# Sachin-A/TraceWeaver

Measured on AMD Instinct MI355X. Metric: spans/sec reconstructed + assignment accuracy vs ground truth, higher is better.
Workload: dtype int64 timestamps, f64 scores; 1 GPU; media_microservices shape (6 services, E in {1,1,1,1,2,4}), 100000 requests/service x 16 replicas per GPU, concurrency 1.6, two-pass reconstruction, device mixture refit; spans_per_gpu=25600000, spans_total=25600000, parallelism=units sharded, 1 rank(s), backend none

## Files before the change

include/traceweaver_amd.h:

```cpp
#ifndef TRACEWEAVER_AMD_H
#define TRACEWEAVER_AMD_H

#include <stdint.h>

#ifdef __cplusplus
extern "C" {
#endif

#define TW_MAX_EP 8
#define TW_TOPK 5
#define TW_MAX_COMP 5
#define TW_MAX_WINDOW 32
#define TW_CAND_WORDS 2
#define TW_SKIP_BASE 1024
#define TW_SKIP_STRIDE 128

typedef enum {
    TW_OK = 0,
    TW_ERR_ARG = -1,
    TW_ERR_UNSUPPORTED = -2,
    TW_ERR_DEVICE = -3,
    TW_ERR_STATE = -4,
    TW_ERR_WINDOW_WIDTH = -5,
    TW_ERR_WINDOW_SIZE = -6,
// ... 50 lines not shown
    int64_t gaps_count;
    int32_t device;
} tw_device_view;
int tw_device_buffers(tw_engine *e, tw_device_view *out);
int tw_set_gaps_device(tw_engine *e, const double *dev_gaps);

int tw_set_mixtures(tw_engine *e, const int32_t *mix_n, const double *mix_p);

#define TW_FIT_ROW_TAPE 34
int tw_fit_mixtures(tw_engine *e);
int tw_fit_mixtures_seeded(tw_engine *e, const uint32_t *unit_seed);
int tw_set_fit_seed(tw_engine *e, uint32_t seed);
int tw_fit_rows(tw_engine *e, int32_t *max_n);
int tw_fit_mixtures_tape(tw_engine *e, const double *tape, int64_t tape_len, const int64_t *slot_off);

int tw_get_mixtures(tw_engine *e, int32_t *mix_n, double *mix_p);

int tw_run_pass2(tw_engine *e);

typedef struct {
    int32_t *parent;
    int32_t *topk_idx;
    double *topk_score;
    int32_t *topk_n;
    int32_t *chosen;
    int64_t *leaves;
    uint8_t *window_end;
    int64_t *unit_stats;
} tw_results;
int tw_get_results(tw_engine *e, int pass, const tw_results *r);
// ... 187 lines not shown
```

traceweaver_amd/_ffi.py:

```python
import ctypes
import os

_HERE = os.path.dirname(os.path.abspath(__file__))
DEFAULT_LIB = os.path.join(_HERE, "lib", "libtwgpu.so")

TW_MAX_EP = 8
TW_TOPK = 5
TW_MAX_COMP = 5

STATUS = {0: "TW_OK", -1: "TW_ERR_ARG", -2: "TW_ERR_UNSUPPORTED", -3: "TW_ERR_DEVICE", -4: "TW_ERR_STATE",
          -5: "TW_ERR_WINDOW_WIDTH", -6: "TW_ERR_WINDOW_SIZE", -7: "TW_ERR_NAN_PARAMS", -8: "TW_ERR_SKIP_PARAMS",
          -9: "TW_ERR_SKIP_REFERENCE_RAISES"}
TW_SKIP_BASE = 1024
TW_SKIP_STRIDE = 128

c_i32p = ctypes.POINTER(ctypes.c_int32)
c_i64p = ctypes.POINTER(ctypes.c_int64)
c_u8p = ctypes.POINTER(ctypes.c_uint8)
c_f64p = ctypes.POINTER(ctypes.c_double)


class Batch(ctypes.Structure):
    _fields_ = [
        ("n_units", ctypes.c_int32),
# ... 92 lines not shown

class ClassProfile(ctypes.Structure):
    _fields_ = [(k, ctypes.c_void_p) for k in (
        "rows", "span_time", "span_min", "span_max", "self_time", "path_time", "path_rows", "path_trees", "offset",
        "class_counted", "class_latency", "class_path_time", "class_top_entry")]


TW_TREE_CONFIDENT = 8
TW_CONF_MAX_EDGES = 15
TW_DIST_MAX_Q = 32
TW_DIST_MAX_EDGES = 63
TW_CMP_MAX_Q = 8
TW_CMP_MAX_PAIRS = 64

EXPORTS = ["tw_create", "tw_destroy", "tw_last_error", "tw_load_batch", "tw_run_pass1", "tw_get_gaps", "tw_set_gaps",
           "tw_device_buffers", "tw_set_gaps_device", "tw_set_mixtures", "tw_fit_mixtures", "tw_fit_mixtures_seeded", "tw_set_fit_seed", "tw_fit_rows", "tw_fit_mixtures_tape", "tw_get_mixtures", "tw_run_pass2", "tw_get_results", "tw_get_gauss_params", "tw_get_timing",
           "tw_assign_service", "tw_find_order", "tw_order_bound", "tw_order_stage", "tw_order_load", "tw_set_truth", "tw_evaluate", "tw_measure_hbm_copy", "tw_host_alloc", "tw_host_free", "tw_build_distributions", "tw_scale_load", "tw_run_baseline", "tw_wap5_delays", "tw_wap5_parents",
           "tw_set_span_rows", "tw_set_parents", "tw_stitch_traces", "tw_set_row_groups", "tw_attribute_traces",
           "tw_get_decisions", "tw_score_traces", "tw_set_row_cohorts", "tw_latency_distributions", "tw_compare_cohorts", "tw_trace_signatures", "tw_class_profiles",
           "tw_corpus_create", "tw_corpus_destroy", "tw_corpus_last_error", "tw_corpus_add_files", "tw_corpus_set_callers", "tw_corpus_counts",
           "tw_corpus_string", "tw_corpus_loop_origin", "tw_corpus_trace_names", "tw_corpus_span_table", "tw_corpus_build_units"]


def load(path=None):
    path = path or DEFAULT_LIB
    if os.environ.get("TW_SET_HW_QUEUES", "0") not in ("", "0"):
        os.environ.setdefault("GPU_MAX_HW_QUEUES", "12")
    if not os.path.exists(path):
        raise ImportError(
            "traceweaver_amd: %s is missing -- build it with `python -c 'import __graft_entry__ as g; g.build()'` "
            "(hipcc --offload-arch=gfx950).  There is no CPU fallback." % path)
# ... 9 lines not shown
    lib.tw_get_gaps.argtypes = [vp, vp]
    lib.tw_set_gaps.argtypes = [vp, vp]
    lib.tw_run_baseline.argtypes = [vp, ctypes.c_int, vp]
    lib.tw_wap5_delays.argtypes = [vp, vp, vp, vp]
    lib.tw_wap5_parents.argtypes = [vp, vp, vp, vp]
    lib.tw_device_buffers.argtypes = [vp, ctypes.POINTER(DeviceView)]
    lib.tw_set_gaps_device.argtypes = [vp, vp]
    lib.tw_scale_load.argtypes = [vp, vp, vp, vp, vp, vp]
    lib.tw_set_mixtures.argtypes = [vp, vp, vp]
    lib.tw_run_pass2.argtypes = [vp]
    lib.tw_fit_mixtures.argtypes = [vp]
    lib.tw_fit_mixtures_seeded.argtypes = [vp, vp]
    lib.tw_set_fit_seed.argtypes = [vp, ctypes.c_uint32]
    lib.tw_fit_rows.argtypes = [vp, vp]
    lib.tw_fit_mixtures_tape.argtypes = [vp, vp, ctypes.c_int64, vp]
    lib.tw_get_mixtures.argtypes = [vp, vp, vp]
    lib.tw_get_results.argtypes = [vp, ctypes.c_int, ctypes.POINTER(Results)]
    lib.tw_get_gauss_params.argtypes = [vp, vp]
    lib.tw_get_timing.argtypes = [vp, vp, ctypes.c_int32]
    lib.tw_assign_service.argtypes = [vp, ctypes.c_int32, vp, vp, ctypes.c_int32, vp, vp, vp, vp, vp, vp, vp,
                                      ctypes.POINTER(Results)]
    lib.tw_find_order.argtypes = [vp, ctypes.c_int32, vp, vp, vp, vp, vp, vp, vp]
    lib.tw_order_bound.argtypes = [vp, ctypes.c_int32, vp, vp, vp, vp, vp, vp, vp, vp]
    lib.tw_order_stage.argtypes = [vp, ctypes.POINTER(Batch)]
    lib.tw_order_load.argtypes = [vp, ctypes.c_int32, vp, vp]
    lib.tw_set_truth.argtypes = [vp, vp, vp, ctypes.c_int64]
    lib.tw_evaluate.argtypes = [vp, vp, vp, vp]
    lib.tw_measure_hbm_copy.argtypes = [vp, ctypes.c_int64, ctypes.c_int32, ctypes.POINTER(ctypes.c_double)]
    lib.tw_build_distributions.argtypes = [vp, ctypes.c_int64, vp, vp, vp, ctypes.c_int64, ctypes.c_int32, vp, vp]
    lib.tw_set_span_rows.argtypes = [vp, ctypes.c_int64, vp, vp, vp, vp, vp, vp]
# ... 34 lines not shown
```

traceweaver_amd/csrc/tw_engine.hip:

```cpp
#include <algorithm>
#include <chrono>
#include <cmath>
#include <cstdio>
#include <cstdlib>
#include <cstring>
#include <functional>
#include <string>
#include <type_traits>
#include <vector>

#include <hip/hip_runtime.h>
#include <rocprim/rocprim.hpp>

#include "traceweaver_amd.h"
#include "tw_kernels.h"
#include "tw_fit.h"
#include "tw_eval.h"
#include "tw_skip.h"
#include "tw_load.h"
#include "tw_baselines.h"
#include "tw_stitch.h"
#include "tw_attr.h"
#include "tw_conf.h"
#include "tw_dist.h"
// ... 27 lines not shown
    int block_params;
    int coop;
    int set_hw_queues;
    int pipeline;
    int sig_hash_bits;
    int debug_lists;
    int stage_min_tiles;
    int tile_sub;
    int lean_pool;
    int split_twins, defer_min_e, lean_min_e, lean_grid, tile_max_deep;
    int64_t part_slots_max;
    int part_budget_deep;
    int fit_sort;
    int stage_gate;
    int fit_spec;
};

Knobs read_knobs() {
    Knobs K;
    K.tile = std::min(std::max(env_int("TW_TILE", kTile), 1), kTile);
    K.tile_threads = std::min(std::max(env_int("TW_TILE_THREADS", 2), 1), 4);
    K.tile_single = env_int("TW_TILE_SINGLE", 1);
    K.tile_single_threads = std::min(std::max(env_int("TW_TILE_SINGLE_THREADS", 1), 1), 4);
    K.tile_pair = env_int("TW_TILE_PAIR", 1);
    K.tile_pair_threads = std::min(std::max(env_int("TW_TILE_PAIR_THREADS", 2), 1), 2);
    K.tile_rank = env_int("TW_TILE_RANK", 1) != 0 ? 1 : 0;
    K.block_params = env_int("TW_BLOCK_PARAMS", 1);
    K.coop = std::min(std::max(env_int("TW_COOP_THREADS", kCoop), 1), kCoop);
    K.set_hw_queues = env_int("TW_SET_HW_QUEUES", 0);
    K.pipeline = env_int("TW_CLASS_PIPELINE", 1);
    K.sig_hash_bits = std::min(std::max(env_int("TW_SIG_HASH_BITS", 64), 1), 64);
    K.debug_lists = env_int("TW_DEBUG_LISTS", 0);
    K.stage_min_tiles = env_int("TW_STAGE_MIN_TILES", 1024);
    K.tile_sub = std::max(env_int("TW_TILE_SUB", 8), 1);
    K.lean_pool = std::min(std::max(env_int("TW_LEAN_POOL", 512), 1), 4096);
    K.split_twins = env_int("TW_SPLIT_TWINS", 2);
    K.defer_min_e = env_int("TW_DEFER_MIN_E", 5);
    K.lean_min_e = env_int("TW_LEAN_MIN_E", 5);
    K.lean_grid = std::max(env_int("TW_LEAN_GRID", TW_LEAN_GRID), 1);
    K.tile_max_deep = std::min(std::max(env_int("TW_TILE_MAX_DEEP", kTileMax), 0), kTileMax);
    K.part_slots_max = (int64_t)std::max(env_int("TW_PART_SLOTS_MAX", 16 << 20), 1024);
    K.part_budget_deep = env_int("TW_PART_BUDGET_DEEP", 2);
    K.fit_sort = env_int("TW_FIT_SORT", 0);
    K.stage_gate = env_int("TW_STAGE_GATE", 1);
    K.fit_spec = env_int("TW_FIT_SPEC", 1) != 0 ? 1 : 0;
    return K;
}

struct Mt19937 {
    uint32_t mt[624];
    int idx = 624;
    explicit Mt19937(uint32_t seed = 0u) {
        mt[0] = seed;
        for (int i = 1; i < 624; i++) mt[i] = 1812433253u * (mt[i - 1] ^ (mt[i - 1] >> 30)) + (uint32_t)i;
    }
    uint32_t next() {
        if (idx >= 624) {
            for (int i = 0; i < 624; i++) {
                const uint32_t y = (mt[i] & 0x80000000u) | (mt[(i + 1) % 624] & 0x7fffffffu);
                mt[i] = mt[(i + 397) % 624] ^ (y >> 1) ^ ((y & 1u) ? 0x9908b0dfu : 0u);
// ... 56 lines not shown
    int32_t *fit_ustart = nullptr, *fit_row_n = nullptr, *fit_row_uniq = nullptr;
    double* fit_centres = nullptr;
    hipEvent_t fit_fork = nullptr, fit_join = nullptr;
    double *fit_spec_centres = nullptr, *fit_spec_p = nullptr;
    int32_t *fit_spec_failed = nullptr, *fit_spec_ctr = nullptr;
    int32_t fit_spec_count[2] = {0, 0};
    double *fit_tape = nullptr, *fit_tape100 = nullptr;
    int64_t* fit_tape_off = nullptr;
    int64_t fit_tape_cap = 0;
    bool fit_runs_pending = false;
    bool fit_prepared = false;
    int32_t hard_pass1[kMaxEp + 1] = {};
    int8_t wide_pass1[kMaxEp + 1] = {};
    int32_t split_pass1[kMaxEp + 1] = {};
    bool pass1_done = false;
    std::vector<int32_t> fit_max_n;
    bool fit_max_n_valid = false;
    Mt19937 fit_rng;
    uint32_t fit_seed = 0;
    int32_t* slot_unit = nullptr;
    int32_t* tile_ids = nullptr;
    int32_t* ctr = nullptr;
    int64_t ctr_round_ints = 0, ctr_pass_ints = 0;
    int32_t tile_cls_off[kMaxEp + 2] = {};
    BlockRef* blk_tab = nullptr;
    int32_t blk_cls_off[kMaxEp + 2] = {};
    uint32_t *seg_gap = nullptr, *seg_gap_end = nullptr, *seg_gap_dst = nullptr;
    unsigned long long *comp_a = nullptr, *comp_b = nullptr;
    int64_t comp_cap = 0, n_gap_scored = 0;
    int32_t *truth = nullptr, *in_trace = nullptr;
    uint8_t* trace_bad = nullptr;
    unsigned long long* eval_counts = nullptr;
// ... 828 lines not shown
    delete e;
}

const char* tw_last_error(const tw_engine* e) { return e ? e->err.c_str() : "null engine"; }

int tw_load_batch(tw_engine* e, const tw_batch* b, int spans_on_device) {
    if (e == nullptr || b == nullptr) return TW_ERR_ARG;
    HIPCHK(hipSetDevice(e->device));
    if (b->n_units <= 0) return fail(e, TW_ERR_ARG, "n_units must be positive");
    if (b->topk != TW_TOPK) return fail(e, TW_ERR_UNSUPPORTED, "topk must be 5 (traceweaver_v3.py:1109)");
    if (b->skip != nullptr && spans_on_device)
        return fail(e, TW_ERR_UNSUPPORTED, "a skip-mode batch takes its span arrays from host memory (spans_on_device = 0)");
    if (b->batch_size <= 0 || b->batch_size_mis <= 0) return fail(e, TW_ERR_ARG, "batch sizes must be positive");
    free_all(e);
    e->fit_rng = Mt19937(e->fit_seed);
    e->fit_prepared = false; e->fit_runs_pending = false; e->fit_max_n_valid = false;
    e->units.assign((size_t)b->n_units, UnitDev{});
    e->tiles.clear();
    e->gs_off_h.assign((size_t)b->n_units, 0);
    int64_t ie = 0, gp = 0, slots = 0, gaps = 0, epi = 0, dagi = 0;
    std::vector<uint32_t> seg_in((size_t)b->n_units + 1), seg_out;
    for (int u = 0; u < b->n_units; u++) {
        UnitDev& U = e->units[(size_t)u];
        const int E = b->unit_E[u];
        const int64_t n = b->unit_in_off[u + 1] - b->unit_in_off[u];
        if (E < 1 || E > TW_MAX_EP) return fail(e, TW_ERR_UNSUPPORTED, "unit has E outside [1, TW_MAX_EP]");
        if (n < 2) return fail(e, TW_ERR_ARG, "a unit needs at least 2 incoming spans (the reference raises on max([]) for 1, traceweaver_v3.py:1119)");
        if (n > (1 << 26)) return fail(e, TW_ERR_ARG, "unit too large (more than 2^26 incoming spans: the selection work lists address a window's first span in 26 bits)");
        U.in_off = b->unit_in_off[u];
        U.tscale = b->unit_time_scale != nullptr ? b->unit_time_scale[u] : 1.0;
        U.float_time = b->unit_time_scale != nullptr ? 1 : 0;
// ... 214 lines not shown
            D.part_used = c + o_pu; D.split_count = c + o_sc; D.err = c + o_err; D.unit_ndirty = c + o_nd;
            D.redo_count = c + o_rd; D.fb_count = c + o_fc; D.defer_refused = c + o_dr; D.fb_total = c + o_ft; D.pair_busy = c + o_pb; D.any_wide = c + o_aw;
            D.unit_stats = (int64_t*)(c + o_us);
        };
        if (e->arena_open) e->arena_req.emplace_back(place, ((size_t)at * sizeof(int32_t) + 255) / 256 * 256);
        else { DEV_ALLOC(e->ctr, at); place(e->ctr); }
    }
    DEV_ALLOC(P.heavy_unit, sel_cap); DEV_ALLOC(P.heavy_win, sel_cap);
    DEV_ALLOC(P.tiny_unit, sel_cap); DEV_ALLOC(P.tiny_win, sel_cap);
    DEV_ALLOC(P.rheavy_unit, sel_cap); DEV_ALLOC(P.rheavy_win, sel_cap); DEV_ALLOC(P.rtiny_unit, sel_cap); DEV_ALLOC(P.rtiny_win, sel_cap);
    DEV_ALLOC(P.hard_unit, sel_cap / (kBruteMax + 1) + 1 + kSelSlots); DEV_ALLOC(P.hard_win, sel_cap / (kBruteMax + 1) + 1 + kSelSlots);
    DEV_ALLOC(e->rank_in, n_in_total); DEV_ALLOC(e->rank_out, n_out_total);
    DEV_ALLOC(e->agg_pair, P.n_tiles); DEV_ALLOC(e->agg_i32, P.n_tiles); DEV_ALLOC(e->agg_i32b, P.n_tiles);
    DEV_ALLOC(e->seg_in, (int64_t)seg_in.size()); DEV_ALLOC(e->seg_out, (int64_t)seg_out.size());
    DEV_ALLOC(e->gaps_sorted, gaps); DEV_ALLOC(e->fit_models, slots * kMaxComp * kModelStride);
    DEV_ALLOC(e->fit_uval, gaps); DEV_ALLOC(e->fit_ustart, gaps); DEV_ALLOC(e->fit_row_n, slots); DEV_ALLOC(e->fit_row_uniq, slots);
    DEV_ALLOC(e->fit_tape, slots * kFitRowTape); DEV_ALLOC(e->fit_tape_off, slots); DEV_ALLOC(e->fit_tape100, kMaxComp * 13);
    e->fit_tape_cap = slots * kFitRowTape;
    DEV_ALLOC(e->fit_centres, slots * kMaxComp * (kMaxComp + 1));
    DEV_ALLOC(e->fit_spec_centres, slots * (kMaxComp + 1)); DEV_ALLOC(e->fit_spec_p, slots * kMaxComp * 3);
    DEV_ALLOC(e->fit_spec_failed, slots); DEV_ALLOC(e->fit_spec_ctr, 2);
    DEV_ALLOC(e->slot_unit, slots); DEV_ALLOC(e->slot_scored, slots);
    DEV_ALLOC(e->seg_gap, (int64_t)seg_gap_h.size()); DEV_ALLOC(e->seg_gap_end, (int64_t)seg_gap_end_h.size()); DEV_ALLOC(e->seg_gap_dst, (int64_t)seg_gap_dst_h.size());
    e->comp_cap = std::max(std::max(n_in_total, n_out_total), e->n_gap_scored);
    DEV_ALLOC(e->comp_a, e->comp_cap); DEV_ALLOC(e->comp_b, e->comp_cap);
    e->skip_mode = b->skip != nullptr;
    std::vector<int32_t> perm_h, pool_h;
    std::vector<int64_t> tw_h;
    std::vector<double> dist_h;
    std::vector<SkipUnitDev> skip_h;
    std::vector<int64_t> sk_tw_off, sk_pool_off, sk_dist_off;
    if (e->skip_mode) {
        perm_h.resize((size_t)n_out_total);
        for (int u = 0; u < b->n_units; u++) {
            const UnitDev& U = e->units[(size_t)u];
            const tw_skip_unit& K = b->skip[u];
// ... 3 lines not shown
                for (int64_t q = 0; q < m; q++) idx[(size_t)q] = (int32_t)q;
                std::stable_sort(idx.begin(), idx.end(), [&](int32_t x, int32_t y) { return b->out_start[a + x] < b->out_start[a + y]; });
                std::copy(idx.begin(), idx.end(), perm_h.begin() + a);
            }
            sk_tw_off.push_back((int64_t)tw_h.size()); sk_pool_off.push_back((int64_t)pool_h.size()); sk_dist_off.push_back((int64_t)dist_h.size());
            tw_h.insert(tw_h.end(), K.tw_start, K.tw_start + K.n_tw);
            pool_h.insert(pool_h.end(), K.pool, K.pool + (int64_t)U.E * K.n_tw);
            dist_h.insert(dist_h.end(), K.dist, K.dist + (int64_t)(U.E + 1) * (U.E + 1) * 2);
        }
        e->skip_fetch_n = (int64_t)pool_h.size();
        DEV_ALLOC(e->skip_units, b->n_units); DEV_ALLOC(e->skip_perm, n_out_total); DEV_ALLOC(e->skip_tw, (int64_t)tw_h.size());
        DEV_ALLOC(e->skip_pool, (int64_t)pool_h.size()); DEV_ALLOC(e->skip_dist, (int64_t)dist_h.size()); DEV_ALLOC(e->skip_fetch, e->skip_fetch_n);
    }
    rc = arena_commit(e);
    if (rc != TW_OK) return rc;
    if (e->skip_mode) {
        for (int u = 0; u < b->n_units; u++) {
            SkipUnitDev K{};
            K.perm = e->skip_perm; K.tw_start = e->skip_tw + sk_tw_off[(size_t)u]; K.pool = e->skip_pool + sk_pool_off[(size_t)u];
            K.dist = e->skip_dist + sk_dist_off[(size_t)u]; K.fetches = e->skip_fetch + sk_pool_off[(size_t)u]; K.n_tw = b->skip[u].n_tw;
            skip_h.push_back(K);
        }
        HIPCHK(hipMemcpyAsync(e->skip_units, skip_h.data(), sizeof(SkipUnitDev) * skip_h.size(), hipMemcpyHostToDevice, e->stream));
        HIPCHK(hipMemcpyAsync(e->skip_perm, perm_h.data(), sizeof(int32_t) * perm_h.size(), hipMemcpyHostToDevice, e->stream));
        HIPCHK(hipMemcpyAsync(e->skip_tw, tw_h.data(), sizeof(int64_t) * tw_h.size(), hipMemcpyHostToDevice, e->stream));
        HIPCHK(hipMemcpyAsync(e->skip_pool, pool_h.data(), sizeof(int32_t) * pool_h.size(), hipMemcpyHostToDevice, e->stream));
        HIPCHK(hipMemcpyAsync(e->skip_dist, dist_h.data(), sizeof(double) * dist_h.size(), hipMemcpyHostToDevice, e->stream));
        HIPCHK(hipStreamSynchronize(e->stream));
    }
    HIPCHK(hipMemsetAsync(P.prof, 0, sizeof(unsigned long long) * 32, e->stream));
// ... 26 lines not shown
    HIPCHK(hipMemsetAsync(P.tk_score, 0xff, sizeof(double) * (size_t)std::max<int64_t>(n_in_total * kTopK, 1), e->stream));
    HIPCHK(hipMemsetAsync(e->mix_n_dev, 0, sizeof(int32_t) * std::max<int64_t>(slots, 1), e->stream));
    HIPCHK(hipStreamSynchronize(e->stream));
    e->scaled_upload = b->unit_time_scale != nullptr;
    e->state = ST_LOADED; e->pass1_done = false;
    for (int E = 0; E <= kMaxEp; E++) { e->wide_pass1[E] = -1; e->hard_pass1[E] = -1; e->split_pass1[E] = -1; }
    return TW_OK;
}

int tw_run_pass1(tw_engine* e) {
    if (e == nullptr) return TW_ERR_ARG;
    if (e->state < ST_LOADED) return fail(e, TW_ERR_STATE, "tw_run_pass1 before tw_load_batch");
    HIPCHK(hipSetDevice(e->device));
    drop_forest(e);
    const int rc = run_pass(e, 1);
    e->fit_prepared = false; e->fit_runs_pending = false; e->fit_max_n_valid = false;
    if (rc == TW_OK) { e->state = ST_PASS1; e->pass1_done = true; }
    return rc;
}

int tw_get_gaps(tw_engine* e, double* gaps) {
    if (e == nullptr || gaps == nullptr) return TW_ERR_ARG;
    if (e->state != ST_PASS1) return fail(e, TW_ERR_STATE, "tw_get_gaps is valid right after tw_run_pass1");
    if (e->skip_mode) return fail(e, TW_ERR_STATE, "a skip-mode batch runs one pass (traceweaver_v3.py:1155-1156): there is no refit");
    HIPCHK(hipSetDevice(e->device));
    HIPCHK(hipMemcpyAsync(gaps, e->P.gaps, sizeof(double) * e->n_gaps, hipMemcpyDeviceToHost, e->stream));
    HIPCHK(hipStreamSynchronize(e->stream));
    return TW_OK;
}

int tw_set_gaps(tw_engine* e, const double* gaps) {
    if (e == nullptr || gaps == nullptr) return TW_ERR_ARG;
    if (e->state < ST_LOADED) return fail(e, TW_ERR_STATE, "tw_set_gaps before tw_load_batch");
    if (e->skip_mode) return fail(e, TW_ERR_STATE, "a skip-mode batch runs one pass (traceweaver_v3.py:1155-1156): there is no refit");
    HIPCHK(hipSetDevice(e->device));
    HIPCHK(hipMemcpyAsync(e->P.gaps, gaps, sizeof(double) * e->n_gaps, hipMemcpyHostToDevice, e->stream));
    HIPCHK(hipStreamSynchronize(e->stream));
    e->fit_prepared = false; e->fit_runs_pending = false; e->fit_max_n_valid = false;
    e->state = ST_PASS1;
    return TW_OK;
}

int tw_device_buffers(tw_engine* e, tw_device_view* out) {
    if (e == nullptr || out == nullptr) return TW_ERR_ARG;
    if (e->state < ST_LOADED) return fail(e, TW_ERR_STATE, "tw_device_buffers before tw_load_batch");
    out->parent = e->P.parent; out->parent_count = e->n_ie;
    out->gaps = e->P.gaps; out->gaps_count = e->n_gaps;
    out->device = e->device;
    return TW_OK;
}

int tw_set_gaps_device(tw_engine* e, const double* dev_gaps) {
    if (e == nullptr || dev_gaps == nullptr) return TW_ERR_ARG;
    if (e->state < ST_LOADED) return fail(e, TW_ERR_STATE, "tw_set_gaps_device before tw_load_batch");
    if (e->skip_mode) return fail(e, TW_ERR_STATE, "a skip-mode batch runs one pass (traceweaver_v3.py:1155-1156): there is no refit");
    HIPCHK(hipSetDevice(e->device));
    HIPCHK(hipMemcpyAsync(e->P.gaps, dev_gaps, sizeof(double) * e->n_gaps, hipMemcpyDeviceToDevice, e->stream));
    HIPCHK(hipStreamSynchronize(e->stream));
    e->fit_prepared = false; e->fit_runs_pending = false; e->fit_max_n_valid = false;
    e->state = ST_PASS1;
    return TW_OK;
}

int tw_set_mixtures(tw_engine* e, const int32_t* mix_n, const double* mix_p) {
    if (e == nullptr || mix_n == nullptr || mix_p == nullptr) return TW_ERR_ARG;
    if (e->state < ST_PASS1) return fail(e, TW_ERR_STATE, "tw_set_mixtures before tw_run_pass1");
    if (e->skip_mode) return fail(e, TW_ERR_STATE, "a skip-mode batch runs one pass (traceweaver_v3.py:1155-1156): there is no second pass");
    HIPCHK(hipSetDevice(e->device));
    for (int64_t q = 0; q < e->n_slots; q++)
        if (mix_n[q] < 0 || mix_n[q] > TW_MAX_COMP) return fail(e, TW_ERR_ARG, "mixture component count outside [0, TW_MAX_COMP]");
    HIPCHK(hipMemcpyAsync(e->mix_n_dev, mix_n, sizeof(int32_t) * e->n_slots, hipMemcpyHostToDevice, e->stream));
    HIPCHK(hipMemcpyAsync(e->mix_p_dev, mix_p, sizeof(double) * e->n_slots * kMaxComp * 3, hipMemcpyHostToDevice, e->stream));
    const int64_t total = e->n_slots * kMaxComp;
    hipLaunchKernelGGL(k_mix_consts, dim3((unsigned)((total + 255) / 256)), dim3(256), 0, e->stream, (const double*)e->mix_p_dev, (const int32_t*)e->mix_n_dev, (const int32_t*)e->slot_unit, e->P.units, e->mix_c_dev, total);
    HIPCHK(hipGetLastError());
    HIPCHK(hipStreamSynchronize(e->stream));
    e->state = ST_MIX;
    return TW_OK;
}

namespace {

FitDev fit_dev(tw_engine* e) {
    FitDev F{};
    F.units = e->P.units; F.n_units = e->P.n_units; F.n_slots = e->n_slots; F.gaps = e->P.gaps; F.sorted = e->gaps_sorted;
    F.gs_off = e->P.gs_off; F.slot_unit = e->slot_unit; F.slot_scored = e->slot_scored; F.models = e->fit_models; F.mix_n = e->mix_n_dev; F.mix_p = e->mix_p_dev;
    F.uval = e->fit_uval; F.ustart = e->fit_ustart; F.row_n = e->fit_row_n; F.row_uniq = e->fit_row_uniq;
    F.tape = e->fit_tape; F.tape_off = e->fit_tape_off; F.tape100 = e->fit_tape100; F.err = e->P.err; F.centres = e->fit_centres;
    F.full_mode = FIT_FINAL; F.spec_centres = e->fit_spec_centres; F.spec_p = e->fit_spec_p; F.spec_failed = e->fit_spec_failed; F.spec_ctr = e->fit_spec_ctr;
    return F;
}

int fit_prepare_launch(tw_engine* e) {
    e->fit_runs_pending = false;
    if (e->fit_prepared || e->K.fit_sort != 0) return TW_OK;
    int32_t* flag = (int32_t*)e->key_acc;
    HIPCHK(hipMemsetAsync(flag, 0, sizeof(int32_t), e->stream));
#ifdef TW_HOST_EMULATION
    const int runs_threads = e->K.coop;
#else
    const int runs_threads = e->K.coop >= 64 ? kRunsThreads : e->K.coop;
#endif
    hipLaunchKernelGGL(k_fit_runs, dim3((unsigned)e->n_slots), dim3(runs_threads), 0, e->stream, fit_dev(e), flag);
    HIPCHK(hipGetLastError());
    e->fit_runs_pending = true;
    return TW_OK;
}
int fit_prepare(tw_engine* e) {
    if (e->fit_prepared) return TW_OK;
    if (e->K.fit_sort == 0) {
        if (!e->fit_runs_pending) { int rl = fit_prepare_launch(e); if (rl != TW_OK) return rl; }
        e->fit_runs_pending = false;
        int32_t* flag = (int32_t*)e->key_acc;
        int32_t refused = 0;
        HIPCHK(hipMemcpyAsync(&refused, flag, sizeof(int32_t), hipMemcpyDeviceToHost, e->stream));
        HIPCHK(hipStreamSynchronize(e->stream));
        if (!refused) {
            e->fit_prepared = true;
            e->fit_max_n_valid = false;
            return TW_OK;
        }
    }
    const unsigned size = (unsigned)e->n_gaps, nseg = (unsigned)e->n_gap_rows;
    unsigned long long kb[2];
    int rck = key_bits(e, e->P.gaps, e->seg_gap, e->seg_gap_end, (int)nseg, e->n_gaps, kb);
    if (rck != TW_OK) return rck;
    unsigned begin_bit = 0;
    if (kb[1] != 0 && !(kb[1] >> 63)) while (!((kb[1] >> begin_bit) & 1)) begin_bit++;
    if (kb[1] >> 63) {
        TWCHK(rocprim_call(e, [&](void* tmp, size_t& bytes) {
            return rocprim::segmented_radix_sort_keys(tmp, bytes, (const double*)e->P.gaps, e->gaps_sorted, size, nseg, e->seg_gap, e->seg_gap_end, 0, 64, e->stream);
        }));
    } else {
        int rcs = sort_rows(e, (const unsigned long long*)e->P.gaps, (unsigned long long*)e->gaps_sorted, size, e->seg_gap, e->seg_gap_end,
                            e->seg_gap_dst, (int)nseg, e->n_gap_scored, begin_bit, 64, 0ull);
        if (rcs != TW_OK) return rcs;
    }
    FitDev F = fit_dev(e);
#ifdef TW_HOST_EMULATION
    const int compress_threads = e->K.coop;
#else
    const int compress_threads = e->K.coop >= 64 ? kCompressThreads : e->K.coop;
#endif
    hipLaunchKernelGGL(k_fit_compress, dim3((unsigned)e->n_slots), dim3(compress_threads), 0, e->stream, F);
    HIPCHK(hipGetLastError());
    e->fit_prepared = true;
    e->fit_max_n_valid = false;
    return TW_OK;
}

int fit_run(tw_engine* e) {
    static const std::vector<double> tape100 = [] {
        std::vector<double> t((size_t)kMaxComp * 13, 0.0);
        for (int k = 1; k <= kMaxComp; k++) {
            Mt19937 r(100u);
            for (int j = 0; j < fit_draws(k); j++) t[(size_t)(k - 1) * 13 + j] = r.random_sample();
        }
        return t;
    }();
    HIPCHK(hipMemcpyAsync(e->fit_tape100, tape100.data(), sizeof(double) * tape100.size(), hipMemcpyHostToDevice, e->stream));
    HIPCHK(hipMemsetAsync(e->P.err, 0, sizeof(int32_t), e->stream));
    FitDev F = fit_dev(e);
    const int threads = e->K.coop >= 64 ? kFitThreads : e->K.coop;
    int side_cls = 0;
    for (int E = kMaxEp; E >= 1; E--)
        if (e->tile_cls_off[E + 1] > e->tile_cls_off[E]) side_cls = E;
    const hipStream_t side = e->cls_stream[side_cls];
    const bool spec = e->K.fit_spec != 0 && side_cls > 0;
    e->fit_spec_count[0] = e->fit_spec_count[1] = 0;
    if (spec) {
        HIPCHK(hipMemsetAsync(e->fit_spec_ctr, 0, 2 * sizeof(int32_t), e->stream));
        HIPCHK(hipEventRecord(e->fit_fork, e->stream));
        HIPCHK(hipStreamWaitEvent(side, e->fit_fork, 0));
        FitDev S = F;
        S.full_mode = FIT_SPEC;
        hipLaunchKernelGGL(k_fit_seed<true>, dim3((unsigned)e->n_slots), dim3(threads), 0, side, S);
        hipLaunchKernelGGL(k_fit_em<true>, dim3((unsigned)e->n_slots), dim3(threads), 0, side, S);
        HIPCHK(hipEventRecord(e->fit_join, side));
    }
    hipLaunchKernelGGL(k_fit_seed<false>, dim3((unsigned)(e->n_slots * (kMaxComp - 1))), dim3(threads), 0, e->stream, F);
    hipLaunchKernelGGL(k_fit_em<false>, dim3((unsigned)(e->n_slots * kMaxComp)), dim3(threads), 0, e->stream, F);
    hipLaunchKernelGGL(k_fit_select, dim3((unsigned)((e->n_slots + 63) / 64)), dim3(64), 0, e->stream, F);
    if (spec) {
        HIPCHK(hipStreamWaitEvent(e->stream, e->fit_join, 0));
        F.full_mode = FIT_ADOPT;
    }
    hipLaunchKernelGGL(k_fit_seed<true>, dim3((unsigned)e->n_slots), dim3(threads), 0, e->stream, F);
    hipLaunchKernelGGL(k_fit_em<true>, dim3((unsigned)e->n_slots), dim3(threads), 0, e->stream, F);
    const int64_t total = e->n_slots * kMaxComp;
    hipLaunchKernelGGL(k_mix_consts, dim3((unsigned)((total + 255) / 256)), dim3(256), 0, e->stream, (const double*)e->mix_p_dev, (const int32_t*)e->mix_n_dev, (const int32_t*)e->slot_unit, e->P.units, e->mix_c_dev, total);
    HIPCHK(hipEventRecord(e->ev[EV_END], e->stream));
    HIPCHK(hipGetLastError());
    int32_t kerr = 0;
    HIPCHK(hipMemcpyAsync(&kerr, e->P.err, sizeof(int32_t), hipMemcpyDeviceToHost, e->stream));
    if (spec) HIPCHK(hipMemcpyAsync(e->fit_spec_count, e->fit_spec_ctr, 2 * sizeof(int32_t), hipMemcpyDeviceToHost, e->stream));
    HIPCHK(hipStreamSynchronize(e->stream));
// ... 17 lines not shown

int tw_set_fit_seed(tw_engine* e, uint32_t seed) {
    if (e == nullptr) return TW_ERR_ARG;
    e->fit_seed = seed;
    e->fit_rng = Mt19937(seed);
    return TW_OK;
}

int tw_fit_rows(tw_engine* e, int32_t* max_n) {
    if (e == nullptr || max_n == nullptr) return TW_ERR_ARG;
    int rc = fit_check_state(e, "tw_fit_rows");
    if (rc != TW_OK) return rc;
    HIPCHK(hipSetDevice(e->device));
    rc = fit_prepare(e);
    if (rc != TW_OK) return rc;
    std::vector<int32_t> uniq((size_t)e->n_slots);
    HIPCHK(hipMemcpyAsync(uniq.data(), e->fit_row_uniq, sizeof(int32_t) * e->n_slots, hipMemcpyDeviceToHost, e->stream));
    HIPCHK(hipStreamSynchronize(e->stream));
    e->fit_max_n.assign((size_t)e->n_slots, 0);
    for (int64_t q = 0; q < e->n_slots; q++) max_n[q] = e->fit_max_n[(size_t)q] = std::min<int32_t>(uniq[(size_t)q], kMaxComp);
    e->fit_max_n_valid = true;
    return TW_OK;
}

int tw_fit_mixtures_tape(tw_engine* e, const double* tape, int64_t tape_len, const int64_t* slot_off) {
    if (e == nullptr || tape == nullptr || slot_off == nullptr || tape_len < 0) return TW_ERR_ARG;
    int rc = fit_check_state(e, "tw_fit_mixtures_tape");
    if (rc != TW_OK) return rc;
    HIPCHK(hipSetDevice(e->device));
    if (!e->fit_prepared || !e->fit_max_n_valid || e->fit_max_n.size() != (size_t)e->n_slots) {
        std::vector<int32_t> tmp((size_t)e->n_slots);
        rc = tw_fit_rows(e, tmp.data());
        if (rc != TW_OK) return rc;
    }
    static const int need[kMaxComp + 1] = {0, 1, 4, 11, 21, 34};
    for (int64_t q = 0; q < e->n_slots; q++) {
        const int m = e->fit_max_n[(size_t)q];
        if (m > 0 && (slot_off[q] < 0 || slot_off[q] + need[m] > tape_len))
            return fail(e, TW_ERR_ARG, "tw_fit_mixtures_tape: the tape does not hold the draws of slot " + std::to_string(q));
    }
    HIPCHK(hipEventRecord(e->ev[EV_BEGIN], e->stream));
    if (tape_len > e->fit_tape_cap) {
        double* p = nullptr;
        rc = dev_alloc(e, &p, tape_len);
        if (rc != TW_OK) return rc;
        e->fit_tape = p;
        e->fit_tape_cap = tape_len;
    }
    HIPCHK(hipMemcpyAsync(e->fit_tape, tape, sizeof(double) * (size_t)std::max<int64_t>(tape_len, 0), hipMemcpyHostToDevice, e->stream));
    HIPCHK(hipMemcpyAsync(e->fit_tape_off, slot_off, sizeof(int64_t) * e->n_slots, hipMemcpyHostToDevice, e->stream));
    return fit_run(e);
}
// ... 90 lines not shown
    for (int i = 0; i < n && i < 6; i++) ms[i] = e->ms[i];
    if (n > 6) ms[6] = e->fit_ms;
    if (n > 7) ms[7] = (double)e->rounds;
    if (n > 8) ms[8] = e->host_ms[0];
    if (n > 9) ms[9] = e->host_ms[1];
    for (int i = 0; i < 6 && 10 + i < n; i++) ms[10 + i] = e->st_ms[i];
    for (int i = 0; i < 3 && 16 + i < n; i++) ms[16 + i] = e->at_ms[i];
    for (int i = 0; i < 3 && 19 + i < n; i++) ms[19 + i] = e->cf_ms[i];
    for (int i = 0; i < 3 && 22 + i < n; i++) ms[22 + i] = e->ds_ms[i];
    for (int i = 0; i < 3 && 25 + i < n; i++) ms[25 + i] = e->sg_ms[i];
    for (int i = 0; i < 3 && 28 + i < n; i++) ms[28 + i] = e->pf_ms[i];
    if (n > 31) ms[31] = e->ob_ms;
    if (n > 32) ms[32] = (double)e->gate_waits;
    for (int i = 0; i < 2 && 33 + i < n; i++) ms[33 + i] = e->cm_ms[i];
    for (int i = 0; i < 2 && 35 + i < n; i++) ms[35 + i] = (double)e->fit_spec_count[i];
    return TW_OK;
}

int tw_debug_profile_hist(tw_engine* e, unsigned long long* out16) {
    if (e == nullptr || out16 == nullptr || e->state < ST_LOADED) return TW_ERR_ARG;
    HIPCHK(hipMemcpyAsync(out16, e->P.prof + 16, sizeof(unsigned long long) * 16, hipMemcpyDeviceToHost, e->stream));
    HIPCHK(hipStreamSynchronize(e->stream));
    return TW_OK;
}

int tw_debug_profile(tw_engine* e, unsigned long long* out16) {
    if (e == nullptr || out16 == nullptr || e->state < ST_LOADED) return TW_ERR_ARG;
    HIPCHK(hipMemcpyAsync(out16, e->P.prof, sizeof(unsigned long long) * 16, hipMemcpyDeviceToHost, e->stream));
    HIPCHK(hipStreamSynchronize(e->stream));
    return TW_OK;
// ... 1393 lines not shown
```

traceweaver_amd/csrc/tw_fit.h:

```cpp
#pragma once
#include "tw_device.h"

namespace tw {

#ifndef TW_FIT_THREADS
#define TW_FIT_THREADS 512
#endif
constexpr int kFitThreads = TW_FIT_THREADS;
constexpr int kFitWaves = kFitThreads / 64;
constexpr int kFitStats = 3 * kMaxComp + 2;
constexpr int kFitMaxIter = 100;
constexpr double kFitTol = 1.0e-3;
constexpr double kFitRegCovar = 1.0e-6;
constexpr int kKmMaxIter = 300;
constexpr double kKmTol = 1.0e-4;
constexpr double kEps10 = 10.0 * 2.220446049250313e-16;
constexpr int kModelStride = 1 + 3 * kMaxComp;
constexpr int kFitMaxTrials = 3;
constexpr int kFitRowTape = 34;

__host__ __device__ inline int fit_trials(int k) { return k < 3 ? 2 : 3; }
__host__ __device__ inline int fit_draws(int k) { return 1 + (k - 1) * fit_trials(k); }
__host__ __device__ inline int fit_tape_pos(int k) { return k == 1 ? 0 : k == 2 ? 1 : k == 3 ? 4 : k == 4 ? 11 : 21; }

// ... 11 lines not shown
    int32_t* row_n;
    int32_t* row_uniq;
    double* models;
    int32_t* mix_n;
    double* mix_p;
    const double* tape;
    const int64_t* tape_off;
    const double* tape100;
    int32_t* err;
    double* centres;
    int32_t full_mode;
    double* spec_centres;
    double* spec_p;
    int32_t* spec_failed;
    int32_t* spec_ctr;
};
enum { FIT_FINAL = 0,
       FIT_SPEC = 1,
       FIT_ADOPT = 2 };

template <int cnt>
__device__ inline void block_reduce(double (&vals)[cnt], double* sh, int nt) {
    const int t = threadIdx.x;
    const int lane = t & 63, wave = t >> 6, nwave = (nt + 63) >> 6;
#pragma unroll
    for (int c = 0; c < cnt; c++) {
        double v = vals[c];
        for (int off = 32; off >= 1; off >>= 1)
            if (off < nt) v += __shfl_down(v, off);
        if (lane == 0) sh[c * kFitWaves + wave] = v;
// ... 189 lines not shown

struct FitRow {
    int64_t q, row;
    int k, n_all, n, uniq;
    bool live;
    bool adopt;
};
__device__ __forceinline__ int fit_spec_k(const FitDev& F, int64_t q) {
    if (!F.slot_scored[q] || F.row_n[q] <= 0) return 0;
    const int u = F.row_uniq[q];
    return u < kMaxComp ? u : kMaxComp;
}
template <bool kFull>
__device__ __forceinline__ FitRow fit_row(const FitDev& F, bool skip1) {
    FitRow R;
    R.q = kFull ? (int64_t)blockIdx.x : (int64_t)(blockIdx.x % F.n_slots);
    R.adopt = false;
    if (kFull) {
        const int sk = F.full_mode != FIT_FINAL ? fit_spec_k(F, R.q) : 0;
        R.k = F.full_mode == FIT_SPEC ? sk : F.mix_n[R.q];
        R.adopt = F.full_mode == FIT_ADOPT && R.k == sk;
    } else {
        R.k = kMaxComp - (int)(blockIdx.x / F.n_slots);
    }
    const UnitDev& U = F.units[F.slot_unit[R.q]];
    R.n_all = U.n_in;
    R.row = F.gs_off[F.slot_unit[R.q]] + (R.q - U.slot_off) * (int64_t)R.n_all;
    R.n = F.row_n[R.q];
    R.uniq = F.row_uniq[R.q];
    R.live = F.slot_scored[R.q] && R.n > 0 && R.k >= (skip1 ? 2 : 1) && R.k <= R.uniq && R.k <= kMaxComp;
    return R;
}

template <bool kFull>
__global__ void __launch_bounds__(kFitThreads) TW_FIT_SEED_ATTR k_fit_seed(FitDev F) {
    __shared__ double sh[(2 * kMaxComp + 1) * kFitWaves];
    __shared__ double cen[kMaxComp];
    __shared__ double blk[kFitWaves][kSeedBlocks];
// ... 505 lines not shown
```

traceweaver_amd/engine.py:

```python
import ctypes
import os
import warnings

import numpy as np

from . import _ffi


class EngineError(RuntimeError):
    def __init__(self, code, message):
        super().__init__("%s (%d): %s" % (_ffi.STATUS.get(code, "TW_ERR"), code, message))
        self.code = code


class UnitArrays(object):

    AFTER_CUT, BEFORE_CUT = 1, 2

    def __init__(self, in_start, in_end, out_off, out_start, out_end, dag, key_rank=None, time_scale=None, part=0):
        self.time_scale = None if time_scale is None else float(time_scale)
        self.part = int(part)
        self.in_start = np.ascontiguousarray(in_start, dtype=np.int64)
        self.in_end = np.ascontiguousarray(in_end, dtype=np.int64)
        self.out_off = np.ascontiguousarray(out_off, dtype=np.int64)
# ... 190 lines not shown
            if seed is not None:
                self._check(self._lib.tw_set_fit_seed(self._h, int(seed)))
            self._check(self._lib.tw_fit_mixtures(self._h))
            return
        t = np.ascontiguousarray(tape, dtype=np.float64)
        o = np.ascontiguousarray(np.concatenate([np.asarray(a, dtype=np.int64).ravel() for a in slot_off]), dtype=np.int64)
        if len(o) != self._slot_off[-1]:
            raise ValueError("tape offsets do not match the loaded batch")
        self._check(self._lib.tw_fit_mixtures_tape(self._h, _vp(t), len(t), _vp(o)))

    def fit_rows(self):
        m = np.empty(int(self._slot_off[-1]), dtype=np.int32)
        self._check(self._lib.tw_fit_rows(self._h, _vp(m)))
        return [m[self._slot_off[k]:self._slot_off[k + 1]] for k in range(len(self.units))]

    def mixtures(self):
        n = np.empty(int(self._slot_off[-1]), dtype=np.int32)
        p = np.empty((int(self._slot_off[-1]), _ffi.TW_MAX_COMP, 3), dtype=np.float64)
        self._check(self._lib.tw_get_mixtures(self._h, _vp(n), _vp(p)))
        return [(n[self._slot_off[k]:self._slot_off[k + 1]], p[self._slot_off[k]:self._slot_off[k + 1]])
                for k in range(len(self.units))]

    def gauss_params(self):
        g = np.empty((int(self._gp_off[-1]), 3), dtype=np.float64)
        self._check(self._lib.tw_get_gauss_params(self._h, _vp(g)))
        return [g[self._gp_off[k]:self._gp_off[k + 1]].reshape(self._nblk[k], u.nslot, 3) for k, u in enumerate(self.units)]

    _FIELDS = ("parent", "topk_idx", "topk_score", "topk_n", "chosen", "leaves", "window_end", "unit_stats")

    def results(self, which, fields=None):
# ... 467 lines not shown
```

Measured before the change: 1.489 billion spans/s.

## Schedule mixture-fit blocks longest-first by row unique count

Builds a host-side permutation of the fit kernels' block indices that puts the heaviest (row, k) work items first. It ranks by unique count times k and pushes dead rows to the end, then uploads the table and indirects blockIdx through it in seed, EM and select kernels. The aim is to cut tail imbalance in the mixture refit, where long rows launched late leave the GPU underused. In exchange it adds a device-to-host copy of row counts, an always-on stream sync in fit_prepare, host sorting per refit, and an extra indirection load per block.

```diff
diff --git a/include/traceweaver_amd.h b/include/traceweaver_amd.h
--- a/include/traceweaver_amd.h
+++ b/include/traceweaver_amd.h
@@ -88,6 +88,8 @@
 int tw_fit_rows(tw_engine *e, int32_t *max_n);
 int tw_fit_mixtures_tape(tw_engine *e, const double *tape, int64_t tape_len, const int64_t *slot_off);
 
+int tw_get_fit_order(tw_engine *e, int32_t *order_seed, int32_t *order_em, int32_t *order_row, int32_t *present);
+
 int tw_get_mixtures(tw_engine *e, int32_t *mix_n, double *mix_p);
 
 int tw_run_pass2(tw_engine *e);
diff --git a/traceweaver_amd/_ffi.py b/traceweaver_amd/_ffi.py
--- a/traceweaver_amd/_ffi.py
+++ b/traceweaver_amd/_ffi.py
@@ -130,7 +130,7 @@
 TW_CMP_MAX_PAIRS = 64
 
 EXPORTS = ["tw_create", "tw_destroy", "tw_last_error", "tw_load_batch", "tw_run_pass1", "tw_get_gaps", "tw_set_gaps",
-           "tw_device_buffers", "tw_set_gaps_device", "tw_set_mixtures", "tw_fit_mixtures", "tw_fit_mixtures_seeded", "tw_set_fit_seed", "tw_fit_rows", "tw_fit_mixtures_tape", "tw_get_mixtures", "tw_run_pass2", "tw_get_results", "tw_get_gauss_params", "tw_get_timing",
+           "tw_device_buffers", "tw_set_gaps_device", "tw_set_mixtures", "tw_fit_mixtures", "tw_fit_mixtures_seeded", "tw_set_fit_seed", "tw_fit_rows", "tw_fit_mixtures_tape", "tw_get_fit_order", "tw_get_mixtures", "tw_run_pass2", "tw_get_results", "tw_get_gauss_params", "tw_get_timing",
            "tw_assign_service", "tw_find_order", "tw_order_bound", "tw_order_stage", "tw_order_load", "tw_set_truth", "tw_evaluate", "tw_measure_hbm_copy", "tw_host_alloc", "tw_host_free", "tw_build_distributions", "tw_scale_load", "tw_run_baseline", "tw_wap5_delays", "tw_wap5_parents",
            "tw_set_span_rows", "tw_set_parents", "tw_stitch_traces", "tw_set_row_groups", "tw_attribute_traces",
            "tw_get_decisions", "tw_score_traces", "tw_set_row_cohorts", "tw_latency_distributions", "tw_compare_cohorts", "tw_trace_signatures", "tw_class_profiles",
@@ -170,6 +170,7 @@
     lib.tw_set_fit_seed.argtypes = [vp, ctypes.c_uint32]
     lib.tw_fit_rows.argtypes = [vp, vp]
     lib.tw_fit_mixtures_tape.argtypes = [vp, vp, ctypes.c_int64, vp]
+    lib.tw_get_fit_order.argtypes = [vp, vp, vp, vp, ctypes.POINTER(ctypes.c_int32)]
     lib.tw_get_mixtures.argtypes = [vp, vp, vp]
     lib.tw_get_results.argtypes = [vp, ctypes.c_int, ctypes.POINTER(Results)]
     lib.tw_get_gauss_params.argtypes = [vp, vp]
diff --git a/traceweaver_amd/csrc/tw_engine.hip b/traceweaver_amd/csrc/tw_engine.hip
--- a/traceweaver_amd/csrc/tw_engine.hip
+++ b/traceweaver_amd/csrc/tw_engine.hip
@@ -7,6 +7,7 @@
 #include <functional>
 #include <string>
 #include <type_traits>
+#include <utility>
 #include <vector>
 
 #include <hip/hip_runtime.h>
@@ -65,6 +66,7 @@
     int fit_sort;
     int stage_gate;
     int fit_spec;
+    int fit_order;
 };
 
 Knobs read_knobs() {
@@ -95,6 +97,7 @@
     K.fit_sort = env_int("TW_FIT_SORT", 0);
     K.stage_gate = env_int("TW_STAGE_GATE", 1);
     K.fit_spec = env_int("TW_FIT_SPEC", 1) != 0 ? 1 : 0;
+    K.fit_order = env_int("TW_FIT_ORDER", 1) != 0 ? 1 : 0;
     return K;
 }
 
@@ -181,8 +184,11 @@
     int8_t wide_pass1[kMaxEp + 1] = {};
     int32_t split_pass1[kMaxEp + 1] = {};
     bool pass1_done = false;
-    std::vector<int32_t> fit_max_n;
-    bool fit_max_n_valid = false;
+    std::vector<int32_t> fit_rows_h;
+    bool fit_rows_h_valid = false;
+    std::vector<int32_t> fit_order_h;
+    int32_t* fit_order_dev = nullptr;
+    double fit_order_host_ms = 0.0;
     Mt19937 fit_rng;
     uint32_t fit_seed = 0;
     int32_t* slot_unit = nullptr;
@@ -1041,7 +1047,7 @@
     if (b->batch_size <= 0 || b->batch_size_mis <= 0) return fail(e, TW_ERR_ARG, "batch sizes must be positive");
     free_all(e);
     e->fit_rng = Mt19937(e->fit_seed);
-    e->fit_prepared = false; e->fit_runs_pending = false; e->fit_max_n_valid = false;
+    e->fit_prepared = false; e->fit_runs_pending = false; e->fit_rows_h_valid = false;
     e->units.assign((size_t)b->n_units, UnitDev{});
     e->tiles.clear();
     e->gs_off_h.assign((size_t)b->n_units, 0);
@@ -1286,12 +1292,14 @@
     DEV_ALLOC(e->agg_pair, P.n_tiles); DEV_ALLOC(e->agg_i32, P.n_tiles); DEV_ALLOC(e->agg_i32b, P.n_tiles);
     DEV_ALLOC(e->seg_in, (int64_t)seg_in.size()); DEV_ALLOC(e->seg_out, (int64_t)seg_out.size());
     DEV_ALLOC(e->gaps_sorted, gaps); DEV_ALLOC(e->fit_models, slots * kMaxComp * kModelStride);
-    DEV_ALLOC(e->fit_uval, gaps); DEV_ALLOC(e->fit_ustart, gaps); DEV_ALLOC(e->fit_row_n, slots); DEV_ALLOC(e->fit_row_uniq, slots);
+    DEV_ALLOC(e->fit_uval, gaps); DEV_ALLOC(e->fit_ustart, gaps); DEV_ALLOC(e->fit_row_n, 2 * slots + 1);
     DEV_ALLOC(e->fit_tape, slots * kFitRowTape); DEV_ALLOC(e->fit_tape_off, slots); DEV_ALLOC(e->fit_tape100, kMaxComp * 13);
     e->fit_tape_cap = slots * kFitRowTape;
     DEV_ALLOC(e->fit_centres, slots * kMaxComp * (kMaxComp + 1));
     DEV_ALLOC(e->fit_spec_centres, slots * (kMaxComp + 1)); DEV_ALLOC(e->fit_spec_p, slots * kMaxComp * 3);
     DEV_ALLOC(e->fit_spec_failed, slots); DEV_ALLOC(e->fit_spec_ctr, 2);
+    DEV_ALLOC(e->fit_order_dev, slots * (2 * kMaxComp));
+    e->fit_order_h.clear();
     DEV_ALLOC(e->slot_unit, slots); DEV_ALLOC(e->slot_scored, slots);
     DEV_ALLOC(e->seg_gap, (int64_t)seg_gap_h.size()); DEV_ALLOC(e->seg_gap_end, (int64_t)seg_gap_end_h.size()); DEV_ALLOC(e->seg_gap_dst, (int64_t)seg_gap_dst_h.size());
     e->comp_cap = std::max(std::max(n_in_total, n_out_total), e->n_gap_scored);
@@ -1325,6 +1333,7 @@
     }
     rc = arena_commit(e);
     if (rc != TW_OK) return rc;
+    e->fit_row_uniq = e->fit_row_n + slots;
     if (e->skip_mode) {
         for (int u = 0; u < b->n_units; u++) {
             SkipUnitDev K{};
@@ -1381,7 +1390,7 @@
     HIPCHK(hipSetDevice(e->device));
     drop_forest(e);
     const int rc = run_pass(e, 1);
-    e->fit_prepared = false; e->fit_runs_pending = false; e->fit_max_n_valid = false;
+    e->fit_prepared = false; e->fit_runs_pending = false; e->fit_rows_h_valid = false;
     if (rc == TW_OK) { e->state = ST_PASS1; e->pass1_done = true; }
     return rc;
 }
@@ -1403,7 +1412,7 @@
     HIPCHK(hipSetDevice(e->device));
     HIPCHK(hipMemcpyAsync(e->P.gaps, gaps, sizeof(double) * e->n_gaps, hipMemcpyHostToDevice, e->stream));
     HIPCHK(hipStreamSynchronize(e->stream));
-    e->fit_prepared = false; e->fit_runs_pending = false; e->fit_max_n_valid = false;
+    e->fit_prepared = false; e->fit_runs_pending = false; e->fit_rows_h_valid = false;
     e->state = ST_PASS1;
     return TW_OK;
 }
@@ -1424,7 +1433,7 @@
     HIPCHK(hipSetDevice(e->device));
     HIPCHK(hipMemcpyAsync(e->P.gaps, dev_gaps, sizeof(double) * e->n_gaps, hipMemcpyDeviceToDevice, e->stream));
     HIPCHK(hipStreamSynchronize(e->stream));
-    e->fit_prepared = false; e->fit_runs_pending = false; e->fit_max_n_valid = false;
+    e->fit_prepared = false; e->fit_runs_pending = false; e->fit_rows_h_valid = false;
     e->state = ST_PASS1;
     return TW_OK;
 }
@@ -1442,6 +1451,7 @@
     hipLaunchKernelGGL(k_mix_consts, dim3((unsigned)((total + 255) / 256)), dim3(256), 0, e->stream, (const double*)e->mix_p_dev, (const int32_t*)e->mix_n_dev, (const int32_t*)e->slot_unit, e->P.units, e->mix_c_dev, total);
     HIPCHK(hipGetLastError());
     HIPCHK(hipStreamSynchronize(e->stream));
+    e->fit_order_h.clear();
     e->state = ST_MIX;
     return TW_OK;
 }
@@ -1461,7 +1471,7 @@
 int fit_prepare_launch(tw_engine* e) {
     e->fit_runs_pending = false;
     if (e->fit_prepared || e->K.fit_sort != 0) return TW_OK;
-    int32_t* flag = (int32_t*)e->key_acc;
+    int32_t* flag = e->fit_row_n + 2 * e->n_slots;
     HIPCHK(hipMemsetAsync(flag, 0, sizeof(int32_t), e->stream));
 #ifdef TW_HOST_EMULATION
     const int runs_threads = e->K.coop;
@@ -1473,18 +1483,21 @@
     e->fit_runs_pending = true;
     return TW_OK;
 }
+int fit_rows_to_host(tw_engine* e) {
+    e->fit_rows_h.resize((size_t)(2 * e->n_slots + 1));
+    HIPCHK(hipMemcpyAsync(e->fit_rows_h.data(), e->fit_row_n, sizeof(int32_t) * e->fit_rows_h.size(), hipMemcpyDeviceToHost, e->stream));
+    return TW_OK;
+}
 int fit_prepare(tw_engine* e) {
     if (e->fit_prepared) return TW_OK;
     if (e->K.fit_sort == 0) {
         if (!e->fit_runs_pending) { int rl = fit_prepare_launch(e); if (rl != TW_OK) return rl; }
         e->fit_runs_pending = false;
-        int32_t* flag = (int32_t*)e->key_acc;
-        int32_t refused = 0;
-        HIPCHK(hipMemcpyAsync(&refused, flag, sizeof(int32_t), hipMemcpyDeviceToHost, e->stream));
+        TWCHK(fit_rows_to_host(e));
         HIPCHK(hipStreamSynchronize(e->stream));
-        if (!refused) {
+        if (!e->fit_rows_h[(size_t)(2 * e->n_slots)]) {
             e->fit_prepared = true;
-            e->fit_max_n_valid = false;
+            e->fit_rows_h_valid = true;
             return TW_OK;
         }
     }
@@ -1511,9 +1524,47 @@
 #endif
     hipLaunchKernelGGL(k_fit_compress, dim3((unsigned)e->n_slots), dim3(compress_threads), 0, e->stream, F);
     HIPCHK(hipGetLastError());
+    TWCHK(fit_rows_to_host(e));
+    HIPCHK(hipStreamSynchronize(e->stream));
     e->fit_prepared = true;
-    e->fit_max_n_valid = false;
-    return TW_OK;
+    e->fit_rows_h_valid = true;
+    return TW_OK;
+}
+
+void fit_order(const int32_t* row_uniq, const int32_t* row_n, int64_t n_slots, std::vector<int32_t>& out) {
+    out.resize((size_t)(n_slots * 2 * kMaxComp));
+    std::vector<int32_t> rows;
+    rows.reserve((size_t)n_slots);
+    for (int64_t q = 0; q < n_slots; q++)
+        if (row_n[q] > 0 && row_uniq[q] >= 1) rows.push_back((int32_t)q);
+    std::stable_sort(rows.begin(), rows.end(), [&](int32_t a, int32_t b) { return row_uniq[a] > row_uniq[b]; });
+    int64_t len[kMaxComp + 1];
+    for (int k = 1; k <= kMaxComp; k++)
+        len[k] = std::partition_point(rows.begin(), rows.end(), [&](int32_t q) { return row_uniq[q] >= k; }) - rows.begin();
+    const auto merge = [&](int32_t* tab, int k_min) {
+        int64_t at = 0, pos[kMaxComp + 1] = {};
+        for (;;) {
+            int best = 0;
+            int64_t best_key = -1;
+            for (int k = kMaxComp; k >= k_min; k--) {
+                if (pos[k] >= len[k]) continue;
+                const int64_t key = (int64_t)row_uniq[rows[(size_t)pos[k]]] * k;
+                if (key > best_key) { best_key = key; best = k; }
+            }
+            if (best == 0) break;
+            tab[at++] = (int32_t)((kMaxComp - best) * n_slots + rows[(size_t)pos[best]++]);
+        }
+        for (int k = kMaxComp; k >= k_min; k--)
+            for (int64_t q = 0; q < n_slots; q++)
+                if (!(row_n[q] > 0 && k <= row_uniq[q])) tab[at++] = (int32_t)((kMaxComp - k) * n_slots + q);
+    };
+    merge(out.data(), 2);
+    merge(out.data() + n_slots * (kMaxComp - 1), 1);
+    int32_t* tab = out.data() + n_slots * (2 * kMaxComp - 1);
+    int64_t at = 0;
+    for (const int32_t q : rows) tab[at++] = q;
+    for (int64_t q = 0; q < n_slots; q++)
+        if (!(row_n[q] > 0 && row_uniq[q] >= 1)) tab[at++] = (int32_t)q;
 }
 
 int fit_run(tw_engine* e) {
@@ -1529,6 +1580,19 @@
     HIPCHK(hipMemsetAsync(e->P.err, 0, sizeof(int32_t), e->stream));
     FitDev F = fit_dev(e);
     const int threads = e->K.coop >= 64 ? kFitThreads : e->K.coop;
+    const int32_t *order_seed = nullptr, *order_em = nullptr, *order_row = nullptr;
+    e->fit_order_h.clear();
+    e->fit_order_host_ms = 0.0;
+    if (e->K.fit_order != 0) {
+        if (!e->fit_rows_h_valid) return fail(e, TW_ERR_STATE, "refit: the rows' counts are not on the host (fit_prepare leaves them there)");
+        const auto h0 = std::chrono::steady_clock::now();
+        fit_order(e->fit_rows_h.data() + e->n_slots, e->fit_rows_h.data(), e->n_slots, e->fit_order_h);
+        HIPCHK(hipMemcpyAsync(e->fit_order_dev, e->fit_order_h.data(), sizeof(int32_t) * e->fit_order_h.size(), hipMemcpyHostToDevice, e->stream));
+        e->fit_order_host_ms = std::chrono::duration<double, std::milli>(std::chrono::steady_clock::now() - h0).count();
+        order_seed = e->fit_order_dev;
+        order_em = order_seed + e->n_slots * (kMaxComp - 1);
+        order_row = order_em + e->n_slots * kMaxComp;
+    }
     int side_cls = 0;
     for (int E = kMaxEp; E >= 1; E--)
         if (e->tile_cls_off[E + 1] > e->tile_cls_off[E]) side_cls = E;
@@ -1541,12 +1605,16 @@
         HIPCHK(hipStreamWaitEvent(side, e->fit_fork, 0));
         FitDev S = F;
         S.full_mode = FIT_SPEC;
+        S.order = order_row;
         hipLaunchKernelGGL(k_fit_seed<true>, dim3((unsigned)e->n_slots), dim3(threads), 0, side, S);
         hipLaunchKernelGGL(k_fit_em<true>, dim3((unsigned)e->n_slots), dim3(threads), 0, side, S);
         HIPCHK(hipEventRecord(e->fit_join, side));
     }
+    F.order = order_seed;
     hipLaunchKernelGGL(k_fit_seed<false>, dim3((unsigned)(e->n_slots * (kMaxComp - 1))), dim3(threads), 0, e->stream, F);
+    F.order = order_em;
     hipLaunchKernelGGL(k_fit_em<false>, dim3((unsigned)(e->n_slots * kMaxComp)), dim3(threads), 0, e->stream, F);
+    F.order = order_row;
     hipLaunchKernelGGL(k_fit_select, dim3((unsigned)((e->n_slots + 63) / 64)), dim3(64), 0, e->stream, F);
     if (spec) {
         HIPCHK(hipStreamWaitEvent(e->stream, e->fit_join, 0));
@@ -1594,12 +1662,20 @@
     HIPCHK(hipSetDevice(e->device));
     rc = fit_prepare(e);
     if (rc != TW_OK) return rc;
-    std::vector<int32_t> uniq((size_t)e->n_slots);
-    HIPCHK(hipMemcpyAsync(uniq.data(), e->fit_row_uniq, sizeof(int32_t) * e->n_slots, hipMemcpyDeviceToHost, e->stream));
-    HIPCHK(hipStreamSynchronize(e->stream));
-    e->fit_max_n.assign((size_t)e->n_slots, 0);
-    for (int64_t q = 0; q < e->n_slots; q++) max_n[q] = e->fit_max_n[(size_t)q] = std::min<int32_t>(uniq[(size_t)q], kMaxComp);
-    e->fit_max_n_valid = true;
+    for (int64_t q = 0; q < e->n_slots; q++) max_n[q] = std::min<int32_t>(e->fit_rows_h[(size_t)(e->n_slots + q)], kMaxComp);
+    return TW_OK;
+}
+
+int tw_get_fit_order(tw_engine* e, int32_t* order_seed, int32_t* order_em, int32_t* order_row, int32_t* present) {
+    if (e == nullptr || order_seed == nullptr || order_em == nullptr || order_row == nullptr || present == nullptr) return TW_ERR_ARG;
+    if (e->state < ST_MIX) return fail(e, TW_ERR_STATE, "tw_get_fit_order: no refit has run on the resident batch");
+    *present = e->fit_order_h.empty() ? 0 : 1;
+    if (*present) {
+        const size_t ns = (size_t)e->n_slots, k = (size_t)kMaxComp;
+        std::copy_n(e->fit_order_h.data(), ns * (k - 1), order_seed);
+        std::copy_n(e->fit_order_h.data() + ns * (k - 1), ns * k, order_em);
+        std::copy_n(e->fit_order_h.data() + ns * (2 * k - 1), ns, order_row);
+    }
     return TW_OK;
 }
 
@@ -1608,14 +1684,11 @@
     int rc = fit_check_state(e, "tw_fit_mixtures_tape");
     if (rc != TW_OK) return rc;
     HIPCHK(hipSetDevice(e->device));
-    if (!e->fit_prepared || !e->fit_max_n_valid || e->fit_max_n.size() != (size_t)e->n_slots) {
-        std::vector<int32_t> tmp((size_t)e->n_slots);
-        rc = tw_fit_rows(e, tmp.data());
-        if (rc != TW_OK) return rc;
-    }
+    rc = fit_prepare(e);
+    if (rc != TW_OK) return rc;
     static const int need[kMaxComp + 1] = {0, 1, 4, 11, 21, 34};
     for (int64_t q = 0; q < e->n_slots; q++) {
-        const int m = e->fit_max_n[(size_t)q];
+        const int m = std::min<int32_t>(e->fit_rows_h[(size_t)(e->n_slots + q)], kMaxComp);
         if (m > 0 && (slot_off[q] < 0 || slot_off[q] + need[m] > tape_len))
             return fail(e, TW_ERR_ARG, "tw_fit_mixtures_tape: the tape does not hold the draws of slot " + std::to_string(q));
     }
@@ -1736,6 +1809,7 @@
     if (n > 32) ms[32] = (double)e->gate_waits;
     for (int i = 0; i < 2 && 33 + i < n; i++) ms[33 + i] = e->cm_ms[i];
     for (int i = 0; i < 2 && 35 + i < n; i++) ms[35 + i] = (double)e->fit_spec_count[i];
+    if (n > 37) ms[37] = e->fit_order_host_ms;
     return TW_OK;
 }
 
diff --git a/traceweaver_amd/csrc/tw_fit.h b/traceweaver_amd/csrc/tw_fit.h
--- a/traceweaver_amd/csrc/tw_fit.h
+++ b/traceweaver_amd/csrc/tw_fit.h
@@ -49,6 +49,7 @@
     double* spec_p;
     int32_t* spec_failed;
     int32_t* spec_ctr;
+    const int32_t* order;
 };
 enum { FIT_FINAL = 0,
        FIT_SPEC = 1,
@@ -268,14 +269,15 @@
 template <bool kFull>
 __device__ __forceinline__ FitRow fit_row(const FitDev& F, bool skip1) {
     FitRow R;
-    R.q = kFull ? (int64_t)blockIdx.x : (int64_t)(blockIdx.x % F.n_slots);
+    const unsigned b = F.order ? (unsigned)F.order[blockIdx.x] : blockIdx.x;
+    R.q = kFull ? (int64_t)b : (int64_t)(b % F.n_slots);
     R.adopt = false;
     if (kFull) {
         const int sk = F.full_mode != FIT_FINAL ? fit_spec_k(F, R.q) : 0;
         R.k = F.full_mode == FIT_SPEC ? sk : F.mix_n[R.q];
         R.adopt = F.full_mode == FIT_ADOPT && R.k == sk;
     } else {
-        R.k = kMaxComp - (int)(blockIdx.x / F.n_slots);
+        R.k = kMaxComp - (int)(b / F.n_slots);
     }
     const UnitDev& U = F.units[F.slot_unit[R.q]];
     R.n_all = U.n_in;
diff --git a/traceweaver_amd/engine.py b/traceweaver_amd/engine.py
--- a/traceweaver_amd/engine.py
+++ b/traceweaver_amd/engine.py
@@ -228,6 +228,13 @@
         self._check(self._lib.tw_fit_rows(self._h, _vp(m)))
         return [m[self._slot_off[k]:self._slot_off[k + 1]] for k in range(len(self.units))]
 
+    def fit_order(self):
+        s = int(self._slot_off[-1])
+        seed, em, row = np.empty(4 * s, dtype=np.int32), np.empty(5 * s, dtype=np.int32), np.empty(s, dtype=np.int32)
+        present = ctypes.c_int32(0)
+        self._check(self._lib.tw_get_fit_order(self._h, _vp(seed), _vp(em), _vp(row), ctypes.byref(present)))
+        return (seed, em, row) if present.value else None
+
     def mixtures(self):
         n = np.empty(int(self._slot_off[-1]), dtype=np.int32)
         p = np.empty((int(self._slot_off[-1]), _ffi.TW_MAX_COMP, 3), dtype=np.float64)
```

Measured after the change: 1.563 billion spans/s (median of 6 runs). 1.05x the previous value.
